# sakarias88/racer-tracer

Hardware: NVIDIA B200
Metric: samples/sec (higher is better)
Workload: dtype f32

## Files before the change

racer_tracer_b200/csrc/rc_api.cu:

```cuda
#include "../../include/racer_cuda.h"

#include <cmath>
#include <cstdio>
#include <cstdlib>
#include <cstring>
#include <chrono>
#include <map>
#include <string>
#include <thread>
#include <vector>

#include "rt_kernels.cuh"
#include "rt_wavefront.cuh"
#include <algorithm>

#include "rc_multi.cuh"
#include "rc_lbvh.cuh"
#include "rc_spec.cuh"

namespace {

thread_local std::string g_last_error;

int fail(int status, const std::string& msg) {
// ... 49 lines not shown
    cudaStream_t stream = nullptr;
    bool own_stream = true;
    cudaEvent_t ev0 = nullptr, ev1 = nullptr;
    cudaEvent_t ev_traced = nullptr;
    DevBuf<int> cancel_word;
    cudaStream_t cancel_stream = nullptr;
    DevBuf<DevPrim> prims;
    DevBuf<DevPrim> prims_lin;
    DevBuf<DevNode> nodes;
    DevBuf<DevTexture> textures;
    DevBuf<DevInstance> instances;
    DevBuf<float4> perlin;
    DevBuf<uint8_t> perm;
    DevBuf<DevPrimD> prims_d;
    DevBuf<int> prim_kind;
    DevBuf<uint32_t> prim_id;
    DevBuf<DevNodeD> nodes_d;
    DevBuf<int> prim_inst;
    DevBuf<DevInstanceD> instances_d;
    std::vector<cudaArray_t> arrays;
    std::vector<std::pair<int, int>> array_dims;
    std::vector<cudaTextureObject_t> tex;
    DevBuf<float> accum;
    DevBuf<float> slice_buf;
    DevBuf<double> out64;
    DevBuf<double> pp_in, pp_mapped;
    DevBuf<uint8_t> pp_rgba;
    DevBuf<unsigned long long> counter;
    DevBuf<uint8_t> ad_active;
    DevBuf<int> ad_spp;
    DevBuf<float> ad_m2;
    DevBuf<double> ad_s2, ad_err;
    WavefrontState wf;
    std::map<std::string, SpecKernel> spec_cache;
    int sm_count = 0, clock_khz = 0;
};

}

struct rc_frame {
    float* base = nullptr;
    size_t image_floats = 0;
    int* words = nullptr;
    int width = 0, height = 0, rank = 0, world = 1;
    int frame_no = 0;
    bool owner = false;
    int* timed_out = nullptr;
// ... 161 lines not shown
    if (!instanced && s->n_prims <= RT_MAX_CONST_PRIMS && rects_fit) mode = RT_MODE_CONST_LINEAR;
    else if (s->n_nodes > 0 && bvh_bytes + perlin_bytes <= RC_SMEM_STAGE_LIMIT) mode = RT_MODE_SMEM_BVH;
    else if (s->n_nodes > 0) mode = RT_MODE_GLOBAL_BVH;
    else mode = RT_MODE_SMEM_LINEAR;
    if (force && !instanced) {
        std::string f(force);
        if (f == "const" && s->n_prims <= RT_MAX_CONST_PRIMS && rects_fit) mode = RT_MODE_CONST_LINEAR;
        else if (f == "smem" && s->n_nodes > 0) mode = RT_MODE_SMEM_BVH;
        else if (f == "global" && s->n_nodes > 0) mode = RT_MODE_GLOBAL_BVH;
        else if (f == "smemlin") mode = RT_MODE_SMEM_LINEAR;
    }
    smem_bytes = perlin_bytes;
    if (mode == RT_MODE_SMEM_BVH) smem_bytes += bvh_bytes;
    if (mode == RT_MODE_SMEM_LINEAR || mode == RT_MODE_CONST_LINEAR) smem_bytes += (size_t)s->n_prims * sizeof(DevPrim);
    return mode;
}

template <typename K>
int set_smem(K kernel, size_t bytes) {
    if (bytes > 48 * 1024) CUDA_TRY(cudaFuncSetAttribute(kernel, cudaFuncAttributeMaxDynamicSharedMemorySize, (int)bytes));
    return RC_OK;
}

template <int MODE, bool TEX>
int launch_mega_mode(const KParams& kp, float* accum, int sampler, int rounds, int blocks, size_t smem, cudaStream_t st) {
#define RC_LAUNCH(S, R)                                                                         \
    do {                                                                                        \
        int rc__ = set_smem(megakernel_render<MODE, S, R, TEX>, smem);                          \
        if (rc__ != RC_OK) return rc__;                                                         \
        megakernel_render<MODE, S, R, TEX><<<blocks, RT_BLOCK, smem, st>>>(kp, accum);          \
    } while (0)
    if (rounds == 7) { if (sampler == RC_SAMPLER_REJECTION) RC_LAUNCH(1, 7); else RC_LAUNCH(0, 7); }
    else { if (sampler == RC_SAMPLER_REJECTION) RC_LAUNCH(1, 10); else RC_LAUNCH(0, 10); }
#undef RC_LAUNCH
    CUDA_TRY(cudaGetLastError());
    return RC_OK;
}

template <int MODE, bool TEX>
int launch_moments_mode(const KParams& kp, float* accum, int blocks, size_t smem, cudaStream_t st, const uint8_t* active, float* round_m2) {
    int rc = set_smem(megakernel_moments<MODE, TEX>, smem);
    if (rc != RC_OK) return rc;
    megakernel_moments<MODE, TEX><<<blocks, RT_BLOCK, smem, st>>>(kp, accum, active, round_m2);
    CUDA_TRY(cudaGetLastError());
    return RC_OK;
}

int launch_mega(int mode, bool tex, const KParams& kp, float* accum, int sampler, int rounds, int blocks, size_t smem, cudaStream_t st,
                const uint8_t* active = nullptr, float* round_m2 = nullptr) {
#define RC_MODE(M) (!active ? (tex ? launch_mega_mode<M, true>(kp, accum, sampler, rounds, blocks, smem, st)          \
                                   : launch_mega_mode<M, false>(kp, accum, sampler, rounds, blocks, smem, st))        \
                             : (tex ? launch_moments_mode<M, true>(kp, accum, blocks, smem, st, active, round_m2)     \
                                    : launch_moments_mode<M, false>(kp, accum, blocks, smem, st, active, round_m2)))
    switch (mode) {
    case RT_MODE_CONST_LINEAR: return RC_MODE(RT_MODE_CONST_LINEAR);
    case RT_MODE_SMEM_BVH: return RC_MODE(RT_MODE_SMEM_BVH);
    case RT_MODE_GLOBAL_BVH: return RC_MODE(RT_MODE_GLOBAL_BVH);
    default: return RC_MODE(RT_MODE_SMEM_LINEAR);
    }
#undef RC_MODE
}

int check_params(const rc_params* p) {
    if (!p) return fail(RC_ERR_INVALID, "params is NULL");
    if (p->width < 2 || p->height < 2) return fail(RC_ERR_INVALID, "width and height must be >= 2 (u = x/(W-1), cpu.rs:35-40)");
    if (p->samples < 1) return fail(RC_ERR_INVALID, "samples must be >= 1");
    if (p->max_depth < 0) return fail(RC_ERR_INVALID, "max_depth must be >= 0");
    if (p->world < 0 || p->rank < 0 || (p->world > 0 && p->rank >= p->world)) return fail(RC_ERR_INVALID, "bad rank/world");
    if (p->rng_rounds != 0 && p->rng_rounds != 7 && p->rng_rounds != 10) return fail(RC_ERR_INVALID, "rng_rounds must be 0, 7 or 10");
    if ((long long)p->width * p->height > (1 << 24)) return fail(RC_ERR_INVALID, "more than 2^24 pixels (RNG counter layout)");
    if (p->samples > (1 << 24)) return fail(RC_ERR_INVALID, "more than 2^24 samples per pixel (RNG counter layout)");
    if (p->max_depth > 63) return fail(RC_ERR_INVALID, "max_depth > 63 (RNG counter layout)");
    if (p->variant != RC_VARIANT_MEGAKERNEL && p->variant != RC_VARIANT_WAVEFRONT) return fail(RC_ERR_INVALID, "unknown variant");
    if (p->sampler != RC_SAMPLER_DIRECT && p->sampler != RC_SAMPLER_REJECTION) return fail(RC_ERR_INVALID, "unknown sampler");
    if (p->split != RC_SPLIT_TILES && p->split != RC_SPLIT_SAMPLES) return fail(RC_ERR_INVALID, "unknown split");
    if (p->specialize < 0 || p->specialize > 2) return fail(RC_ERR_INVALID, "specialize must be 0, 1 or 2");
    if (!(p->tile_w == 0 && p->tile_h == 0) && !(p->tile_w == RT_TILE_W && p->tile_h == RT_TILE_H))
        return fail(RC_ERR_INVALID, "tile_w x tile_h must be 0 x 0 or 16 x 8 (the kernels' tile is fixed)");
    return RC_OK;
}

void set_vstep(KParams& kp, int screen_height) {
    const double s = 1.0 / ((double)(screen_height - 1) * 65536.0);
    kp.vstep = make_float4((float)(kp.cam.vertical.x * s), (float)(kp.cam.vertical.y * s), (float)(kp.cam.vertical.z * s), 0.0f);
}

void partition(KParams& kp, const rc_params* p, int part, int parts) {
    kp.width = p->width; kp.height = p->height;
    kp.max_depth = p->max_depth;
    kp.fixed_jitter = p->fixed_jitter;
    kp.key = (uint32_t)p->seed ^ (uint32_t)(p->seed >> 32);
    for (int r = 0; r < 10; ++r) kp.ks[r] = kp.key + (uint32_t)r * PHILOX2_W;
    kp.inv_wm1 = 1.0f / (float)(p->width - 1); kp.inv_hm1 = 1.0f / (float)(p->height - 1);
    kp.wm1 = (float)(p->width - 1);
    set_vstep(kp, p->height);
    kp.px_scale_x = kp.px_scale_y = 1;
    kp.tile_w = RT_TILE_W; kp.tile_h = RT_TILE_H;
    kp.slices = 1; kp.slice_buf = nullptr;
    kp.overwrite = 0;
    kp.final_scale = 0.0f;
    kp.tiles_x = (p->width + RT_TILE_W - 1) / RT_TILE_W;
    int tiles_y = (p->height + RT_TILE_H - 1) / RT_TILE_H;
    int total = kp.tiles_x * tiles_y;
    if (p->split == RC_SPLIT_SAMPLES) {
        kp.tile_first = 0; kp.tile_stride = 1; kp.n_tiles = total;
        long long lo = (long long)p->samples * part / parts, hi = (long long)p->samples * (part + 1) / parts;
        kp.s_begin = (int)lo; kp.s_end = (int)hi;
    } else {
        kp.tile_first = part; kp.tile_stride = parts;
        kp.n_tiles = part < total ? (total - part + parts - 1) / parts : 0;
        kp.s_begin = 0; kp.s_end = p->samples;
    }
}

bool cancelled(const volatile int32_t* cancel) { return cancel && *cancel != 0; }

bool direct_tiles(const rc_ctx* ctx, const rc_params* p) {
    return ctx->devs.size() > 1 && p->split == RC_SPLIT_TILES && ctx->multi.peer_write_ok && p->variant == RC_VARIANT_MEGAKERNEL;
}

struct AdaptiveRound {
    const uint8_t* active;
    float* round_m2;
    int s_begin, s_end;
};

struct ShareCall {
    float* accum0;
    const volatile int32_t* cancel;
    bool store = false;
    float final_scale = 0.0f;
    bool spread_stores = false;
    int preview_sw = 0, preview_sh = 0, preview_w = 0, preview_h = 0;
    const AdaptiveRound* round = nullptr;
};

int trace_share(rc_ctx* ctx, const rc_params* p, const ShareCall& call, bool& was_cancelled) {
    was_cancelled = false;
    const int n_dev = (int)ctx->devs.size();
    const int world = p->world > 0 ? p->world : 1;
    const int parts = world * n_dev;
    const int rounds = p->rng_rounds ? p->rng_rounds : 10;
    const bool direct = direct_tiles(ctx, p);
    uint64_t launches = 0;
    bool used_spec = false;
    for (int k = 0; k < n_dev; ++k) {
        DeviceState& d = ctx->devs[k];
        CUDA_TRY(cudaSetDevice(d.device));
        if (k == 0) {
            if (!call.round) CUDA_TRY(cudaEventRecord(d.ev0, d.stream));
            if (n_dev > 1) CUDA_TRY(cudaEventRecord(d.ev_traced, d.stream));
        } else {
            CUDA_TRY(cudaStreamWaitEvent(d.stream, ctx->devs[0].ev_traced, 0));
        }
        if (!call.round) CUDA_TRY(cudaMemsetAsync(d.counter.p, 0, sizeof(unsigned long long), d.stream));
    }
    const bool relay = call.cancel != nullptr && p->variant == RC_VARIANT_MEGAKERNEL;
    if (relay)
// ... 38 lines not shown
            continue;
        }
        SpecKernel* spec = nullptr;
        const bool spec_mode_ok = ctx->smem_bytes <= 48 * 1024 &&
                                  (ctx->mode == RT_MODE_CONST_LINEAR ||
                                   ((ctx->mode == RT_MODE_SMEM_BVH || ctx->mode == RT_MODE_GLOBAL_BVH) && std::getenv("RC_NO_BVH_SPEC") == nullptr));
        if (p->specialize && spec_mode_ok && p->sampler == RC_SAMPLER_DIRECT && !p->fixed_jitter) {
            std::string err;
            if (!spec_load_api((const void*)&rc_abi_version)) err = spec_api().err;
            else {
                if (ctx->spec_rounds != rounds) { ctx->spec_source.clear(); ctx->spec_source_moments.clear(); }
                std::string& source = call.round ? ctx->spec_source_moments : ctx->spec_source;
                if (source.empty()) {
                    source = spec_generate(ctx->kp, ctx->has_textures, ctx->mats_mask, ctx->mode, ctx->prims_mask, ctx->instanced, rounds,
                                           call.round != nullptr);
                    ctx->spec_rounds = rounds;
                }
                spec = spec_build(d.spec_cache, source, err, ++ctx->spec_clock);
            }
            if (!spec && p->specialize == 1) return fail(RC_ERR_STATE, "scene specialisation failed: " + err);
        } else if (p->specialize == 1) {
            return fail(RC_ERR_INVALID, "specialize = 1 needs the megakernel, the direct sampler and no fixed jitter");
        }
        const int s0 = kp.s_begin, s1 = kp.s_end;
        kp.slices = 1;
        kp.slice_buf = nullptr;
        kp.slice_halving = 0;
        if (!call.round) {
            const long long want = 8LL * d.sm_count * 10;
            long long sl = (want + kp.n_tiles - 1) / kp.n_tiles;
            if (sl > (s1 - s0) / 16) sl = (s1 - s0) / 16;
            if (sl < 2 && s1 - s0 >= 512 && !call.spread_stores) sl = 2;
            if (const char* e = std::getenv("RC_SLICES")) sl = std::atoll(e);
            kp.slice_halving = sl >= 5 ? 1 : 0;
            if (const char* e = std::getenv("RC_SLICE_HALVING")) kp.slice_halving = std::atoi(e);
            while (kp.slice_halving && sl > 1 && ((s1 - s0) >> (sl - 1)) < 8) --sl;
            if (sl > 1) {
                CUDA_TRY(d.slice_buf.resize((size_t)sl * kp.n_tiles * RT_BLOCK * 3));
                kp.slices = (int)sl;
                kp.slice_buf = d.slice_buf.p;
            }
        }
        {
            int rc = RC_ERR_CUDA;
            if (spec) {
                rc = spec_launch(spec, kp, accum, kp.n_tiles * kp.slices, ctx->smem_bytes, d.stream, active, round_m2) == 0 ? RC_OK : RC_ERR_CUDA;
                if (rc == RC_OK) used_spec = true;
                else if (p->specialize == 1) return fail(rc, "launch of the scene-specialised kernel failed");
            }
            if (rc != RC_OK)
                rc = launch_mega(ctx->mode, ctx->has_textures, kp, accum, p->sampler, rounds, kp.n_tiles * kp.slices, ctx->smem_bytes, d.stream,
                                 active, round_m2);
            if (rc != RC_OK) return rc;
            ++launches;
            if (kp.slices > 1) {
                reduce_slices_kernel<<<(kp.n_tiles * RT_BLOCK + 255) / 256, 256, 0, d.stream>>>(kp, accum);
                CUDA_TRY(cudaGetLastError());
                ++launches;
            }
        }
        if (relay) CUDA_TRY(cudaEventRecord(d.ev_traced, d.stream));
    }
    ctx->stats.kernel_launches = launches;
    ctx->stats.specialized = used_spec ? 1 : 0;
    if (relay) {
        for (;;) {
            bool done = true;
            for (int k = 0; k < n_dev && done; ++k) {
                const cudaError_t e = cudaEventQuery(ctx->devs[k].ev_traced);
                if (e == cudaErrorNotReady) done = false;
                else if (e != cudaSuccess) return fail(RC_ERR_CUDA, std::string("cudaEventQuery: ") + cudaGetErrorString(e));
            }
            if (!was_cancelled && cancelled(call.cancel)) {
                was_cancelled = true;
                for (int k = 0; k < n_dev; ++k) {
                    DeviceState& d = ctx->devs[k];
                    CUDA_TRY(cudaSetDevice(d.device));
                    CUDA_TRY(cudaMemcpyAsync(d.cancel_word.p, ctx->cancel_relay, sizeof(int), cudaMemcpyHostToDevice, d.cancel_stream));
                }
// ... 459 lines not shown
    for (int k = 0; k < n; ++k) {
        DeviceState& d = ctx->devs[k];
        d.device = devices ? devices[k] : k;
        if (d.device < 0 || d.device >= count) {
            delete ctx;
            return fail(RC_ERR_NO_DEVICE, "device ordinal out of range");
        }
        cudaError_t err = cudaSetDevice(d.device);
        if (err == cudaSuccess) err = cudaStreamCreateWithFlags(&d.stream, cudaStreamNonBlocking);
        if (err == cudaSuccess) err = cudaEventCreate(&d.ev0);
        if (err == cudaSuccess) err = cudaEventCreate(&d.ev1);
        if (err == cudaSuccess) err = cudaEventCreateWithFlags(&d.ev_traced, cudaEventDisableTiming);
        if (err == cudaSuccess) err = d.counter.resize(1);
        cudaDeviceProp prop;
        if (err == cudaSuccess) err = cudaGetDeviceProperties(&prop, d.device);
        if (err != cudaSuccess) {
            delete ctx;
            return fail(RC_ERR_CUDA, std::string("device setup failed: ") + cudaGetErrorString(err));
        }
        d.sm_count = prop.multiProcessorCount;
        d.clock_khz = prop.clockRate;
        {
            cudaFuncAttributes fa;
            cudaFuncGetAttributes(&fa, reduce_slices_kernel);
            cudaFuncGetAttributes(&fa, finalize_kernel);
            cudaFuncGetAttributes(&fa, finalize_to_f64_kernel);
            cudaFuncGetAttributes(&fa, widen_kernel);
            cudaFuncGetAttributes(&fa, frame_wait_kernel);
            cudaFuncGetAttributes(&fa, frame_publish_kernel);
            cudaFuncGetAttributes(&fa, sum_slots_kernel);
            cudaGetLastError();
        }
    }
    ctx->stats.n_devices = n;
    ctx->stats.sm_count = ctx->devs[0].sm_count;
    ctx->stats.sm_clock_khz = ctx->devs[0].clock_khz;
    int rc = multi_init(ctx->multi, ctx->devs.size(), [&](size_t k) { return ctx->devs[k].device; });
    if (rc != RC_OK) {
        delete ctx;
        return fail(rc, "peer access setup failed");
    }
    cudaSetDevice(ctx->devs[0].device);
    if (cudaHostAlloc((void**)&ctx->cancel_relay, sizeof(int), cudaHostAllocPortable) != cudaSuccess) {
        cudaGetLastError();
        rc_destroy(ctx);
        return fail(RC_ERR_CUDA, "cudaHostAlloc of the cancel relay failed");
    }
// ... 4 lines not shown
            cudaGetLastError();
            rc_destroy(ctx);
            return fail(RC_ERR_CUDA, "cudaStreamCreate of the cancel stream failed");
        }
    }
    cudaSetDevice(ctx->devs[0].device);
    *out = ctx;
    return RC_OK;
}

int rc_destroy(rc_ctx* ctx) {
    if (!ctx) return RC_OK;
    cudaSetDevice(ctx->devs.empty() ? 0 : ctx->devs[0].device);
    while (!ctx->frames.empty()) rc_frame_close(ctx, ctx->frames.back());
    for (void* q : ctx->shared_opened) cudaIpcCloseMemHandle(q);
    for (void* q : ctx->shared_owned) cudaFree(q);
    if (ctx->cancel_relay) cudaFreeHost(ctx->cancel_relay);
    multi_destroy(ctx->multi);
    for (auto& d : ctx->devs) {
        cudaSetDevice(d.device);
        cudaDeviceSynchronize();
        free_scene(d);
        free_tables(d);
        d.accum.release(); d.slice_buf.release(); d.out64.release(); d.counter.release(); d.cancel_word.release();
        d.ad_active.release(); d.ad_spp.release(); d.ad_m2.release(); d.ad_s2.release(); d.ad_err.release();
        if (d.cancel_stream) cudaStreamDestroy(d.cancel_stream);
        d.pp_in.release(); d.pp_mapped.release(); d.pp_rgba.release();
        if (d.ev_traced) cudaEventDestroy(d.ev_traced);
        wavefront_release(d.wf);
        spec_release(d.spec_cache);
        if (d.ev0) cudaEventDestroy(d.ev0);
        if (d.ev1) cudaEventDestroy(d.ev1);
        if (d.own_stream && d.stream) cudaStreamDestroy(d.stream);
    }
    delete ctx;
    return RC_OK;
}

int rc_set_stream(rc_ctx* ctx, void* cuda_stream) {
    if (!ctx) return fail(RC_ERR_INVALID, "ctx is NULL");
    DeviceState& d = ctx->devs[0];
    CUDA_TRY(cudaSetDevice(d.device));
    if (d.own_stream && d.stream) CUDA_TRY(cudaStreamDestroy(d.stream));
    d.stream = reinterpret_cast<cudaStream_t>(cuda_stream);
    d.own_stream = false;
    return RC_OK;
}
// ... 268 lines not shown
    if (p->variant != RC_VARIANT_MEGAKERNEL) return fail(RC_ERR_INVALID, "rc_render_frame needs the megakernel");
    const bool by_samples = p->split == RC_SPLIT_SAMPLES;
    if (p->width != f->width || p->height != f->height) return fail(RC_ERR_INVALID, "params and frame sizes differ");
    const int world = p->world > 0 ? p->world : 1;
    if (world != f->world || p->rank != f->rank) return fail(RC_ERR_INVALID, "params and frame rank / world differ");
    if (f->rank != 0 && (d_rgb || out_rgb)) return fail(RC_ERR_INVALID, "only rank 0 receives the image");
    if (ctx->devs.size() != 1) return fail(RC_ERR_INVALID, "rc_render_frame is the one-process-per-GPU form: the context must hold one device");
    if (!ctx->has_scene || !ctx->has_camera) return fail(RC_ERR_STATE, "upload a scene and set a camera first");
    if (cancelled(cancel)) return fail(RC_ERR_CANCELLED, "cancel flag set before the render started");
    if (*f->timed_out) return fail(RC_ERR_STATE, "an earlier frame never completed (a rank stopped publishing progress)");
    DeviceState& d = ctx->devs[0];
    CUDA_TRY(cudaSetDevice(d.device));
    const int frame_no = ++f->frame_no;
    float* image = f->base + (size_t)(frame_no & 1) * f->world * f->image_floats;
    float* target = by_samples ? image + (size_t)f->rank * f->image_floats : image;
    if (world > 1) {
        if (f->rank == 0) frame_publish_kernel<<<1, 1, 0, d.stream>>>(f->words, frame_no + 1);
        else frame_wait_kernel<<<1, 32, 0, d.stream>>>(f->words, 0, 1, frame_no, f->timed_out);
        CUDA_TRY(cudaGetLastError());
    }
    bool was_cancelled = false;
    ShareCall call{target, cancel, true};
    call.final_scale = by_samples ? 0.0f : 1.0f / (float)p->samples;
    call.spread_stores = by_samples && world > 1;
    rc = trace_share(ctx, p, call, was_cancelled);
    if (rc != RC_OK) return rc;
    if (by_samples && (long long)p->samples * (f->rank + 1) / world <= (long long)p->samples * f->rank / world) {
        CUDA_TRY(cudaMemsetAsync(target, 0, f->image_floats * sizeof(float), d.stream));
    }
    uint64_t extra = 0;
    if (world > 1) {
        if (f->rank != 0) { frame_publish_kernel<<<1, 1, 0, d.stream>>>(f->words + 32 * f->rank, frame_no); extra = 2; }
        else { frame_wait_kernel<<<1, 32, 0, d.stream>>>(f->words, 1, world - 1, frame_no, f->timed_out); extra = 2; }
        CUDA_TRY(cudaGetLastError());
    }
    if (by_samples && f->rank == 0) {
        const size_t n = (size_t)p->width * p->height * 3;
        sum_slots_kernel<<<(unsigned)((n + 255) / 256), 256, 0, d.stream>>>(image, f->image_floats, world, n, 1.0f / (float)p->samples);
        CUDA_TRY(cudaGetLastError());
        extra += 1;
    }
    rc = finish_stats(ctx, p);
    if (rc != RC_OK) return rc;
    ctx->stats.kernel_launches += extra;
    if (d_rgb) *d_rgb = image;
    if (out_rgb && !was_cancelled) {
        const size_t n = (size_t)p->width * p->height * 3;
// ... 432 lines not shown
```

racer_tracer_b200/csrc/rc_spec.cuh:

```cuda
#pragma once
#include <cuda_runtime.h>
#include <dlfcn.h>

#include <cmath>
#include <cstdio>
#include <cstdlib>
#include <cstring>
#include <fstream>
#include <map>
#include <sstream>
#include <string>
#include <vector>

#include "rt_kernels.cuh"

struct SpecKernel {
    void* module = nullptr;
    void* function = nullptr;
    std::string source;
    std::string error;
    uint64_t last_use = 0;
};

#define RC_SPEC_CACHE_MAX 8

struct SpecApi {
    bool tried = false, ok = false;
    std::string err;
    void* nvrtc = nullptr;
    void* cuda = nullptr;
    int (*CreateProgram)(void**, const char*, const char*, int, const char* const*, const char* const*) = nullptr;
    int (*CompileProgram)(void*, int, const char* const*) = nullptr;
    int (*GetCUBINSize)(void*, size_t*) = nullptr;
    int (*GetCUBIN)(void*, char*) = nullptr;
    int (*GetProgramLogSize)(void*, size_t*) = nullptr;
    int (*GetProgramLog)(void*, char*) = nullptr;
    int (*DestroyProgram)(void**) = nullptr;
    int (*cuModuleLoadData)(void**, const void*) = nullptr;
    int (*cuModuleGetFunction)(void**, void*, const char*) = nullptr;
    int (*cuModuleUnload)(void*) = nullptr;
    int (*cuLaunchKernel)(void*, unsigned, unsigned, unsigned, unsigned, unsigned, unsigned, unsigned, void*, void**, void**) = nullptr;
    std::string header_dir;
};

inline SpecApi& spec_api() {
    static SpecApi api;
    return api;
}

inline bool spec_load_api(const void* anchor_symbol) {
    SpecApi& a = spec_api();
    if (a.tried) return a.ok;
    a.tried = true;
    const char* nvrtc_names[] = {"libnvrtc.so.12", "libnvrtc.so", "/usr/local/cuda/lib64/libnvrtc.so.12"};
    for (const char* n : nvrtc_names) { a.nvrtc = dlopen(n, RTLD_NOW); if (a.nvrtc) break; }
    if (!a.nvrtc) { a.err = "libnvrtc.so.12 not found"; return false; }
    a.cuda = dlopen("libcuda.so.1", RTLD_NOW);
    if (!a.cuda) { a.err = "libcuda.so.1 not found"; return false; }
#define RC_SYM(lib, field, name)                                                        \
    *(void**)(&a.field) = dlsym(a.lib, name);                                           \
    if (!a.field) { a.err = std::string("missing symbol ") + name; return false; }
    RC_SYM(nvrtc, CreateProgram, "nvrtcCreateProgram");
    RC_SYM(nvrtc, CompileProgram, "nvrtcCompileProgram");
    RC_SYM(nvrtc, GetCUBINSize, "nvrtcGetCUBINSize");
    RC_SYM(nvrtc, GetCUBIN, "nvrtcGetCUBIN");
    RC_SYM(nvrtc, GetProgramLogSize, "nvrtcGetProgramLogSize");
    RC_SYM(nvrtc, GetProgramLog, "nvrtcGetProgramLog");
    RC_SYM(nvrtc, DestroyProgram, "nvrtcDestroyProgram");
    RC_SYM(cuda, cuModuleLoadData, "cuModuleLoadData");
    RC_SYM(cuda, cuModuleGetFunction, "cuModuleGetFunction");
    RC_SYM(cuda, cuModuleUnload, "cuModuleUnload");
    RC_SYM(cuda, cuLaunchKernel, "cuLaunchKernel");
#undef RC_SYM
    Dl_info info;
    if (!dladdr(anchor_symbol, &info) || !info.dli_fname) { a.err = "cannot locate the library on disk"; return false; }
    std::string path(info.dli_fname);
    size_t slash = path.find_last_of('/');
    a.header_dir = (slash == std::string::npos ? std::string(".") : path.substr(0, slash)) + "/csrc/";
    a.ok = true;
    return true;
}

inline int __float_as_int_host(float f) { int i; std::memcpy(&i, &f, sizeof(i)); return i; }

inline std::string spec_float(float v) {
    char buf[64];
    std::snprintf(buf, sizeof(buf), "%.9g", (double)v);
    std::string s(buf);
    if (s.find_first_of(".eEn") == std::string::npos) s += ".0";
    return s + "f";
}

inline std::string spec_entry(const char* mode, int rounds, bool tex, bool moments) {
    std::ostringstream o;
    o << "extern \"C\" __global__ void __launch_bounds__(RT_BLOCK, RT_MIN_BLOCKS)\n"
// ... 393 lines not shown
        return remember_failure();
    }
    size_t n = 0;
    a.GetCUBINSize(prog, &n);
    std::vector<char> cubin(n);
    a.GetCUBIN(prog, cubin.data());
    a.DestroyProgram(&prog);
    SpecKernel k;
    k.source = source;
    k.last_use = now;
    if (a.cuModuleLoadData(&k.module, cubin.data()) != 0) { err = "cuModuleLoadData failed"; return remember_failure(); }
    if (a.cuModuleGetFunction(&k.function, k.module, "spec_megakernel") != 0) { err = "spec_megakernel not found in module"; return remember_failure(); }
    auto res = cache.emplace(source, k);
    return &res.first->second;
}

inline void spec_release(std::map<std::string, SpecKernel>& cache) {
    SpecApi& a = spec_api();
    for (auto& kv : cache)
        if (kv.second.module && a.cuModuleUnload) a.cuModuleUnload(kv.second.module);
    cache.clear();
}

inline int spec_launch(SpecKernel* k, const KParams& kp, float* accum, int blocks, size_t smem, cudaStream_t st,
                       const uint8_t* active = nullptr, float* round_m2 = nullptr) {
    SpecApi& a = spec_api();
    KParams p = kp;
    void* args[4] = {&p, &accum, &active, &round_m2};
    return a.cuLaunchKernel(k->function, (unsigned)blocks, 1, 1, RT_BLOCK, 1, 1, (unsigned)smem, (void*)st, args, nullptr);
}
```

racer_tracer_b200/csrc/rt_kernels.cuh:

```cuda
#pragma once
#include "rt_scene.cuh"

#define RT_TILE_W 16
#define RT_TILE_H 8
#define RT_BLOCK 128

#define RT_MODE_CONST_LINEAR 0
#define RT_MODE_SMEM_BVH 1
#define RT_MODE_GLOBAL_BVH 2
#define RT_MODE_SMEM_LINEAR 3

struct SmemLayout {
    const DevNode* nodes;
    const DevPrim* prims;
    const float4* perlin;
    const uint8_t* perm;
};

template <int MODE>
RT_D SmemLayout stage_scene(const KParams& P, unsigned char* smem) {
    SmemLayout L;
    L.nodes = P.nodes; L.prims = P.prims; L.perlin = P.perlin; L.perm = P.perlin_perm;
    float4* dst = reinterpret_cast<float4*>(smem);
    if (MODE == RT_MODE_SMEM_BVH) {
// ... 231 lines not shown

#ifndef RT_STEAL
#define RT_STEAL 1
#endif
#ifndef RT_STEAL_MIN
#define RT_STEAL_MIN 4
#endif


#ifndef RT_KCONST_MASK
#define RT_KCONST_MASK 7
#endif
#ifndef RT_PHILOX_LATE
#define RT_PHILOX_LATE 0
#endif

RT_D float radiance_y(const vec3f& a, const vec3f& b) { return (a.x * b.x + a.y * b.y + a.z * b.z) * (1.0f / 3.0f); }

template <int MODE, int SAMPLER, int ROUNDS, bool TEX, bool MOMENTS = false>
RT_D void megakernel_body(const KParams& P, float* __restrict__ accum, unsigned char* smem,
                          const uint8_t* __restrict__ active_px = nullptr, float* __restrict__ round_m2 = nullptr) {
    constexpr int PARKED = MOMENTS ? 4 : 3;
    __shared__ float steal_parked[RT_STEAL ? PARKED * RT_BLOCK : 1];
    if (P.cancel_flag != nullptr &&
        __syncthreads_or(threadIdx.x == 0 && *reinterpret_cast<const volatile int*>(P.cancel_flag) != 0)) return;
    bool active = true;
    if constexpr (MOMENTS) {
        const int tile = P.tile_first + (int)blockIdx.x * P.tile_stride;
        const int w = threadIdx.x >> 5, l = threadIdx.x & 31;
        const int x = (tile % P.tiles_x) * RT_TILE_W + (w & 1) * 8 + (l & 7);
        const int y = (tile / P.tiles_x) * RT_TILE_H + (w >> 1) * 4 + (l >> 3);
        active = x < P.width && y < P.height && active_px[y * P.width + x] != 0;
        if (!__syncthreads_or(active ? 1 : 0)) return;
    }
    __shared__ float reg_consts[7];
    if (threadIdx.x == 0) {
        reg_consts[0] = 2.0f; reg_consts[1] = 6.283185307179586f / 16777216.0f; reg_consts[2] = 1.0f;
#ifdef RT_SPECIALIZED
        spec_reg_consts(reg_consts + 3);
#endif
    }
    SmemLayout L = stage_scene<MODE>(P, smem);
    TexCtx X; X.perlin = L.perlin; X.perm = L.perm;
    {
        const volatile float* rc = reg_consts;
        if (RT_KCONST_MASK & 1) X.k_two = rc[0];
        if (RT_KCONST_MASK & 2) X.k_phi = rc[1];
        if (RT_KCONST_MASK & 4) X.k_one = rc[2];
#ifdef RT_SPECIALIZED
#pragma unroll
        for (int j = 0; j < RT_SPEC_REG_CONSTS; ++j) X.k_spec[j] = rc[3 + j];
#endif
    }

    const int slice = P.slices > 1 ? (int)blockIdx.x / P.n_tiles : 0;
    const int tile_k = P.slices > 1 ? (int)blockIdx.x - slice * P.n_tiles : (int)blockIdx.x;
    const int tile = P.tile_first + tile_k * P.tile_stride;
    const int tx = tile % P.tiles_x, ty = tile / P.tiles_x;
    const int warp = threadIdx.x >> 5, lane = threadIdx.x & 31;
    const int px = tx * RT_TILE_W + (warp & 1) * 8 + (lane & 7);
    const int py = ty * RT_TILE_H + (warp >> 1) * 4 + (lane >> 3);
    const bool valid = px < P.width && py < P.height;
    int s_first = P.s_begin, s_last = P.s_end;
    if (P.slices > 1 && P.slice_halving) {
        const int n = P.s_end - P.s_begin;
        s_first = P.s_begin + (n - (n >> slice));
        s_last = slice + 1 == P.slices ? P.s_end : P.s_begin + (n - (n >> (slice + 1)));
    } else if (P.slices > 1) {
        const long long n = P.s_end - P.s_begin, S = P.slices, total = S * (S + 1) / 2;
        const long long c0 = (long long)slice * S - (long long)slice * (slice - 1) / 2;
        const long long c1 = c0 + (S - slice);
        s_first = P.s_begin + (int)(n * c0 / total);
        s_last = P.s_begin + (int)(n * c1 / total);
    }

    PixelCtx pc = pixel_setup<ROUNDS>(P, valid ? px : 0, valid ? py : 0);
    RngCtx R; R.ks = P.ks; R.pixel = pc.pixel; R.sample = 0;
    const uint32_t own_pixel = pc.pixel;
    PhiloxPre ppre = philox2x32_pre(pc.pixel, P.ks);
    uint32_t vj_bits = __byte_perm(0u, 0u, 0);
    {
        const uint2 w = philox2x32_from<ROUNDS>(ppre, rt_ctr1(rt_vjit_sample((uint32_t)s_first), 0u, RT_TAG_PATH), P.ks);
        vj_bits = __byte_perm(w.y, w.x, 0x0040);
    }
    int owner = lane;
    float* const parked = steal_parked + 32 * PARKED * warp;
    if (RT_STEAL) {
        parked[lane] = 0.0f; parked[lane + 32] = 0.0f; parked[lane + 64] = 0.0f;
        if constexpr (MOMENTS) parked[lane + 96] = 0.0f;
        __syncwarp();
    }

    vec3f sum = mk3(0.0f, 0.0f, 0.0f);
    float m2 = 0.0f;
    vec3f o = mk3(0.0f, 0.0f, 0.0f), d = o, T = o;
    const vec3f T_ONE = mk3(1.0f, 1.0f, 1.0f);
    float time = 0.0f;
    int s = valid && active ? s_first : s_last;
    float depth_left = 0.0f;
    int last_prim = -1;
    uint32_t seg = 0;
    uint32_t ctr1 = 0;
    unsigned sh_prims = (unsigned)__cvta_generic_to_shared(L.prims);
    asm volatile("" : "+r"(sh_prims));
    unsigned nseg = 0;
    if (P.max_depth <= 0) {
        const float n = (float)(s_last - s);
        sum = mk3(n, n, n);
        if constexpr (MOMENTS) m2 = n;
        s = s_last;
    }

    if (P.tile_cull && (MODE == RT_MODE_CONST_LINEAR || MODE == RT_MODE_SMEM_LINEAR) && P.max_depth > 0) {
        if (!tile_may_hit(P, L.prims, tx, ty)) {
            if (valid) {
                nseg += (unsigned)(s_last - s);
#pragma unroll 1
                for (; s < s_last; ++s) {
                    if (RT_SPEC_BG_BLACK) { s = s_last; break; }
                    vec3f bg;
                    if (__float_as_int(P.bg_a.w) == 0) {
                        const uint2 rnd = philox2x32_ks<ROUNDS>(pc.pixel, rt_ctr1(rt_vjit_sample((uint32_t)s), 0u, RT_TAG_PATH), P.ks);
                        const float vjit = RT_FIXED_JITTER(P) ? 32768.0f : u16lo_int(rnd);
                        camera_ray<SAMPLER, ROUNDS>(P, pc, (uint32_t)s, vjit, o, d, time);
                        bg = background_color(P, d);
                    } else bg = mk3(P.bg_a.x, P.bg_a.y, P.bg_a.z);
                    sum = mk3(fmaf(T_ONE.x, bg.x, sum.x), fmaf(T_ONE.y, bg.y, sum.y), fmaf(T_ONE.z, bg.z, sum.z));
                    if constexpr (MOMENTS) { const float y = radiance_y(T_ONE, bg); m2 = fmaf(y, y, m2); }
                }
            }
            s = s_last;
        }
    }

#ifdef RT_SPEC_SNAP_TABLE
    __syncthreads();
    if ((int)threadIdx.x < P.n_prims) {
        float* row = const_cast<float*>(reinterpret_cast<const float*>(L.prims + threadIdx.x));
        float4 a = make_float4(0.f, 0.f, 0.f, 0.f);
        float bx = 0.f, cw = 0.f;
        spec_snap_row((int)threadIdx.x, a, bx, cw);
        row[0] = a.x; row[1] = a.y; row[2] = a.z; row[3] = a.w; row[4] = bx; row[11] = cw;
    }
    __syncthreads();
#endif

    auto iteration = [&]() {
        const bool fresh = depth_left == 0.0f;
        if (fresh) {
            R.sample = (uint32_t)s;
            ctr1 = R.sample;
            seg = 0; last_prim = -1;
            T = mk3(1.0f, 1.0f, 1.0f);
            depth_left = (float)P.max_depth;
        }
        asm("{\n\t.reg .pred pf;\n\tsetp.ne.s32 pf, %1, 0;\n\t@pf add.s32 %0, %0, 1;\n\t}" : "+r"(s) : "r"((int)fresh));
        if (fresh) {
            const float vjit = RT_FIXED_JITTER(P) ? 32768.0f : (float)(unsigned short)vj_bits;
            camera_ray<SAMPLER, ROUNDS>(P, pc, R.sample, vjit, o, d, time);
        }
#if !RT_PHILOX_LATE
        const uint2 rnd = philox2x32_from<ROUNDS>(ppre, ctr1, P.ks);
        if (fresh) vj_bits = __byte_perm(rnd.y, rnd.x, 0x0040);
#endif
        RayT<float> r = make_ray(o, d, time);
        float t;
        int prim;
        if (MODE == RT_MODE_CONST_LINEAR) { ConstScene S(P, sh_prims); prim = closest_hit<MODE>(P, S, r, last_prim, t, X); }
// ... 85 lines not shown
    }
#undef RT_LANE_BUSY
    if (RT_STEAL) {
        unsigned pending = __ballot_sync(0xffffffffu, owner != lane);
        while (pending) {
            const int l = __ffs(pending) - 1;
            pending &= pending - 1;
            if (lane == l) {
                parked[owner] += sum.x; parked[owner + 32] += sum.y; parked[owner + 64] += sum.z;
                if constexpr (MOMENTS) parked[owner + 96] += m2;
            }
            __syncwarp();
        }
        if (owner != lane) { sum = mk3(0.0f, 0.0f, 0.0f); m2 = 0.0f; }
        sum = mk3(sum.x + parked[lane], sum.y + parked[lane + 32], sum.z + parked[lane + 64]);
        if constexpr (MOMENTS) m2 += parked[lane + 96];
    }
    if constexpr (MOMENTS) {
        if (valid && active) {
            float* a = accum + 3 * (size_t)own_pixel;
            a[0] += sum.x; a[1] += sum.y; a[2] += sum.z;
            round_m2[own_pixel] = m2;
        }
    } else if (P.slices > 1) {
        float* a = P.slice_buf + 3 * ((size_t)slice * ((size_t)P.n_tiles * RT_BLOCK) + (size_t)tile_k * RT_BLOCK + threadIdx.x);
        a[0] = sum.x; a[1] = sum.y; a[2] = sum.z;
    } else if (valid) {
        float* a = accum + 3 * (size_t)own_pixel;
        if (P.final_scale != 0.0f) sum = mk3(sqrtf(P.final_scale * sum.x), sqrtf(P.final_scale * sum.y), sqrtf(P.final_scale * sum.z));
        if (P.overwrite) { a[0] = sum.x; a[1] = sum.y; a[2] = sum.z; }
        else { a[0] += sum.x; a[1] += sum.y; a[2] += sum.z; }
    }
    for (int off = 16; off > 0; off >>= 1) nseg += __shfl_xor_sync(0xffffffffu, nseg, off);
    if (lane == 0 && P.segment_counter) atomicAdd(P.segment_counter, (unsigned long long)nseg);
}

#ifndef RT_SPECIALIZED
__global__ void reduce_slices_kernel(const __grid_constant__ KParams P, float* __restrict__ accum) {
    const int rank = blockIdx.x * blockDim.x + threadIdx.x;
    if (rank >= P.n_tiles * RT_BLOCK) return;
    const int tile_k = rank / RT_BLOCK, within = rank % RT_BLOCK;
    const int tile = P.tile_first + tile_k * P.tile_stride;
    const int tx = tile % P.tiles_x, ty = tile / P.tiles_x;
    const int warp = within >> 5, lane = within & 31;
    const int px = tx * RT_TILE_W + (warp & 1) * 8 + (lane & 7);
    const int py = ty * RT_TILE_H + (warp >> 1) * 4 + (lane >> 3);
    if (px >= P.width || py >= P.height) return;
    float sx = 0.f, sy = 0.f, sz = 0.f;
    for (int j = 0; j < P.slices; ++j) {
        const float* a = P.slice_buf + 3 * ((size_t)j * ((size_t)P.n_tiles * RT_BLOCK) + rank);
        sx += a[0]; sy += a[1]; sz += a[2];
    }
    float* dst = accum + 3 * ((size_t)py * P.width + px);
    if (P.final_scale != 0.0f) { sx = sqrtf(P.final_scale * sx); sy = sqrtf(P.final_scale * sy); sz = sqrtf(P.final_scale * sz); }
    if (P.overwrite) { dst[0] = sx; dst[1] = sy; dst[2] = sz; }
    else { dst[0] += sx; dst[1] += sy; dst[2] += sz; }
}

template <int MODE, int SAMPLER, int ROUNDS, bool TEX>
__global__ void __launch_bounds__(RT_BLOCK, MODE == RT_MODE_GLOBAL_BVH ? RT_MIN_BLOCKS_GLOBAL_BVH : RT_MIN_BLOCKS)
megakernel_render(const __grid_constant__ KParams P, float* __restrict__ accum) {
    extern __shared__ __align__(16) unsigned char smem[];
    megakernel_body<MODE, SAMPLER, ROUNDS, TEX>(P, accum, smem);
}

template <int MODE, bool TEX>
__global__ void __launch_bounds__(RT_BLOCK, MODE == RT_MODE_GLOBAL_BVH ? RT_MIN_BLOCKS_GLOBAL_BVH : RT_MIN_BLOCKS)
megakernel_moments(const __grid_constant__ KParams P, float* __restrict__ accum, const uint8_t* __restrict__ active,
                   float* __restrict__ round_m2) {
    extern __shared__ __align__(16) unsigned char smem[];
    megakernel_body<MODE, 0, 10, TEX, true>(P, accum, smem, active, round_m2);
}

// ... 353 lines not shown
```

racer_tracer_b200/csrc/rt_scene.cuh:

```cuda
#pragma once
#include "rt_math.cuh"

#define RT_PRIM_SPHERE 0
#define RT_PRIM_XY 1
#define RT_PRIM_XZ 2
#define RT_PRIM_YZ 3
#define RT_PRIM_MOVING 4
#define RT_IS_SPHERE(type) (((type) & 3) == 0)
#define RT_MAT_LAMBERTIAN 0
#define RT_MAT_METAL 1
#define RT_MAT_DIELECTRIC 2
#define RT_MAT_LIGHT 3
#define RT_TEX_SOLID 0
#define RT_TEX_CHECKER 1
#define RT_TEX_IMAGE 2
#define RT_TEX_NOISE 3

#ifndef RT_SPEC_PRIMS
#define RT_SPEC_PRIMS 0xF
#endif
#ifndef RT_HAS_INSTANCES
#define RT_HAS_INSTANCES 1
#endif
#define RT_HAS_SPHERES (RT_SPEC_PRIMS & 1)
// ... 43 lines not shown

template <typename T>
struct DevCamera {
    Vec3T<T> origin, upper_left_corner, right, up, horizontal, vertical;
    T lens_radius, time_a, time_b;
};

struct KParams {
    DevCamera<float> cam;
    float4 bg_a, bg_b;
    int width, height;
    float inv_wm1, inv_hm1;
    float wm1;
    float4 vstep;
    int px_scale_x, px_scale_y;
    int s_begin, s_end;
    int max_depth;
    int fixed_jitter;
    uint32_t key;
    uint32_t ks[10];
    int tile_first, tile_stride, n_tiles;
    int overwrite;
    float final_scale;
    int slices;
    int slice_halving;
    float* slice_buf;
    int tiles_x, tile_w, tile_h;
    int n_prims, n_nodes;
    int lin_end[4];
    int n_perlin;
    int checker_depth;
    int lens_enabled;
    int tile_cull;
    int has_motion;
    int ref_aabb;
    const DevPrim* prims;
    const DevPrim* prims_lin;
    const DevNode* nodes;
    const DevTexture* textures;
    const DevInstance* instances;
    const float4* perlin;
    const uint8_t* perlin_perm;
    cudaTextureObject_t images[RT_MAX_IMAGES];
    int image_w[RT_MAX_IMAGES], image_h[RT_MAX_IMAGES];
    unsigned long long* segment_counter;
    const int* cancel_flag;
    DevPrim cprims[RT_MAX_CONST_PRIMS];
    float4 crect_bounds[3][RT_MAX_CONST_RECTS];
    float crect_k[3][RT_MAX_CONST_RECTS];
// ... 743 lines not shown
```

Measured before the change: 65.55 billion.

## Replace static sample slicing with persistent blocks pulling a dynamic work queue

Replaces the fixed per-tile sample slicing with a host-built work list. Tail tiles are split into sample-range pieces, and a persistent grid sized by occupancy takes items through an atomic counter. Each partial piece writes to its own slot, and a reduce-slots kernel sums the slots of cut tiles only. The goal is better load balancing at the tail and less launch and reduction overhead. The cost is an atomic and a block barrier per work item, plus host work-list construction that is cached by a key.

```diff
diff --git a/racer_tracer_b200/csrc/rc_api.cu b/racer_tracer_b200/csrc/rc_api.cu
--- a/racer_tracer_b200/csrc/rc_api.cu
+++ b/racer_tracer_b200/csrc/rc_api.cu
@@ -95,7 +95,10 @@
     std::vector<std::pair<int, int>> array_dims;
     std::vector<cudaTextureObject_t> tex;
     DevBuf<float> accum;
-    DevBuf<float> slice_buf;
+    DevBuf<int4> work;
+    std::vector<int4> work_items, work_cut;
+    int work_slots = 0;
+    long long work_key[5] = {-1, -1, -1, -1, -1};
     DevBuf<double> out64;
     DevBuf<double> pp_in, pp_mapped;
     DevBuf<uint8_t> pp_rgba;
@@ -303,13 +306,19 @@
     return RC_OK;
 }
 
+int persistent_grid(const KParams& kp, int blocks, int per_sm, int sm_count) {
+    return kp.n_items > 0 ? std::min(blocks, std::max(per_sm, 1) * sm_count) : blocks;
+}
+
 template <int MODE, bool TEX>
-int launch_mega_mode(const KParams& kp, float* accum, int sampler, int rounds, int blocks, size_t smem, cudaStream_t st) {
+int launch_mega_mode(const KParams& kp, float* accum, int sampler, int rounds, int blocks, int sm_count, size_t smem, cudaStream_t st) {
 #define RC_LAUNCH(S, R)                                                                         \
     do {                                                                                        \
         int rc__ = set_smem(megakernel_render<MODE, S, R, TEX>, smem);                          \
         if (rc__ != RC_OK) return rc__;                                                         \
-        megakernel_render<MODE, S, R, TEX><<<blocks, RT_BLOCK, smem, st>>>(kp, accum);          \
+        int per_sm__ = 0;                                                                       \
+        CUDA_TRY(cudaOccupancyMaxActiveBlocksPerMultiprocessor(&per_sm__, megakernel_render<MODE, S, R, TEX>, RT_BLOCK, smem)); \
+        megakernel_render<MODE, S, R, TEX><<<persistent_grid(kp, blocks, per_sm__, sm_count), RT_BLOCK, smem, st>>>(kp, accum); \
     } while (0)
     if (rounds == 7) { if (sampler == RC_SAMPLER_REJECTION) RC_LAUNCH(1, 7); else RC_LAUNCH(0, 7); }
     else { if (sampler == RC_SAMPLER_REJECTION) RC_LAUNCH(1, 10); else RC_LAUNCH(0, 10); }
@@ -319,20 +328,23 @@
 }
 
 template <int MODE, bool TEX>
-int launch_moments_mode(const KParams& kp, float* accum, int blocks, size_t smem, cudaStream_t st, const uint8_t* active, float* round_m2) {
+int launch_moments_mode(const KParams& kp, float* accum, int blocks, int sm_count, size_t smem, cudaStream_t st, const uint8_t* active,
+                        float* round_m2) {
     int rc = set_smem(megakernel_moments<MODE, TEX>, smem);
     if (rc != RC_OK) return rc;
-    megakernel_moments<MODE, TEX><<<blocks, RT_BLOCK, smem, st>>>(kp, accum, active, round_m2);
+    int per_sm = 0;
+    CUDA_TRY(cudaOccupancyMaxActiveBlocksPerMultiprocessor(&per_sm, megakernel_moments<MODE, TEX>, RT_BLOCK, smem));
+    megakernel_moments<MODE, TEX><<<persistent_grid(kp, blocks, per_sm, sm_count), RT_BLOCK, smem, st>>>(kp, accum, active, round_m2);
     CUDA_TRY(cudaGetLastError());
     return RC_OK;
 }
 
-int launch_mega(int mode, bool tex, const KParams& kp, float* accum, int sampler, int rounds, int blocks, size_t smem, cudaStream_t st,
-                const uint8_t* active = nullptr, float* round_m2 = nullptr) {
-#define RC_MODE(M) (!active ? (tex ? launch_mega_mode<M, true>(kp, accum, sampler, rounds, blocks, smem, st)          \
-                                   : launch_mega_mode<M, false>(kp, accum, sampler, rounds, blocks, smem, st))        \
-                             : (tex ? launch_moments_mode<M, true>(kp, accum, blocks, smem, st, active, round_m2)     \
-                                    : launch_moments_mode<M, false>(kp, accum, blocks, smem, st, active, round_m2)))
+int launch_mega(int mode, bool tex, const KParams& kp, float* accum, int sampler, int rounds, int blocks, int sm_count, size_t smem,
+                cudaStream_t st, const uint8_t* active = nullptr, float* round_m2 = nullptr) {
+#define RC_MODE(M) (!active ? (tex ? launch_mega_mode<M, true>(kp, accum, sampler, rounds, blocks, sm_count, smem, st)          \
+                                   : launch_mega_mode<M, false>(kp, accum, sampler, rounds, blocks, sm_count, smem, st))        \
+                             : (tex ? launch_moments_mode<M, true>(kp, accum, blocks, sm_count, smem, st, active, round_m2)     \
+                                    : launch_moments_mode<M, false>(kp, accum, blocks, sm_count, smem, st, active, round_m2)))
     switch (mode) {
     case RT_MODE_CONST_LINEAR: return RC_MODE(RT_MODE_CONST_LINEAR);
     case RT_MODE_SMEM_BVH: return RC_MODE(RT_MODE_SMEM_BVH);
@@ -377,7 +389,7 @@
     set_vstep(kp, p->height);
     kp.px_scale_x = kp.px_scale_y = 1;
     kp.tile_w = RT_TILE_W; kp.tile_h = RT_TILE_H;
-    kp.slices = 1; kp.slice_buf = nullptr;
+    kp.n_items = 0; kp.unused0 = 0; kp.work = nullptr;
     kp.overwrite = 0;
     kp.final_scale = 0.0f;
     kp.tiles_x = (p->width + RT_TILE_W - 1) / RT_TILE_W;
@@ -411,10 +423,30 @@
     const volatile int32_t* cancel;
     bool store = false;
     float final_scale = 0.0f;
-    bool spread_stores = false;
     int preview_sw = 0, preview_sh = 0, preview_w = 0, preview_h = 0;
     const AdaptiveRound* round = nullptr;
 };
+
+#define RC_MIN_PIECE 16
+
+void build_work_list(int n_tiles, int s0, int s1, int sm_count, long long forced, std::vector<int4>& items,
+                     std::vector<int4>& cut, int& n_slots) {
+    items.clear(); cut.clear(); n_slots = 0;
+    const long long n = s1 - s0, load = (long long)sm_count * RT_MIN_BLOCKS;
+    const long long tail = forced > 0 ? n_tiles : std::min<long long>(n_tiles, 2 * load);
+    for (int k = 0; k < n_tiles - tail; ++k) items.push_back(make_int4(k, 0, 0, -1));
+    for (long long k = n_tiles - tail; k < n_tiles; ++k) {
+        long long pieces = std::min(forced, n);
+        if (forced <= 0) {
+            const long long piece = std::max<long long>(RC_MIN_PIECE, (n_tiles - k) * n / (2 * load));
+            pieces = std::max<long long>(1, n / piece);
+        }
+        if (pieces <= 1) { items.push_back(make_int4((int)k, 0, 0, -1)); continue; }
+        cut.push_back(make_int4((int)k, n_slots, (int)pieces, 0));
+        for (long long j = 0; j < pieces; ++j)
+            items.push_back(make_int4((int)k, s0 + (int)(n * j / pieces), s0 + (int)(n * (j + 1) / pieces), n_slots++));
+    }
+}
 
 int trace_share(rc_ctx* ctx, const rc_params* p, const ShareCall& call, bool& was_cancelled) {
     was_cancelled = false;
@@ -499,39 +531,43 @@
         } else if (p->specialize == 1) {
             return fail(RC_ERR_INVALID, "specialize = 1 needs the megakernel, the direct sampler and no fixed jitter");
         }
-        const int s0 = kp.s_begin, s1 = kp.s_end;
-        kp.slices = 1;
-        kp.slice_buf = nullptr;
-        kp.slice_halving = 0;
-        if (!call.round) {
-            const long long want = 8LL * d.sm_count * 10;
-            long long sl = (want + kp.n_tiles - 1) / kp.n_tiles;
-            if (sl > (s1 - s0) / 16) sl = (s1 - s0) / 16;
-            if (sl < 2 && s1 - s0 >= 512 && !call.spread_stores) sl = 2;
-            if (const char* e = std::getenv("RC_SLICES")) sl = std::atoll(e);
-            kp.slice_halving = sl >= 5 ? 1 : 0;
-            if (const char* e = std::getenv("RC_SLICE_HALVING")) kp.slice_halving = std::atoi(e);
-            while (kp.slice_halving && sl > 1 && ((s1 - s0) >> (sl - 1)) < 8) --sl;
-            if (sl > 1) {
-                CUDA_TRY(d.slice_buf.resize((size_t)sl * kp.n_tiles * RT_BLOCK * 3));
-                kp.slices = (int)sl;
-                kp.slice_buf = d.slice_buf.p;
+        {
+            long long forced = call.round ? 1 : 0;
+            if (const char* e = std::getenv("RC_SLICES"); e && !call.round) forced = std::atoll(e);
+            const long long key[5] = {kp.n_tiles, forced == 1 ? 0 : kp.s_begin, forced == 1 ? 0 : kp.s_end, d.sm_count, forced};
+            if (!std::equal(key, key + 5, d.work_key)) {
+                build_work_list(kp.n_tiles, kp.s_begin, kp.s_end, d.sm_count, forced, d.work_items, d.work_cut, d.work_slots);
+                const size_t n_items = d.work_items.size(), slot_int4s = (size_t)d.work_slots * RT_BLOCK * 3 / 4;
+                CUDA_TRY(d.work.resize(1 + n_items + slot_int4s + d.work_cut.size()));
+                std::vector<int4> head(1 + n_items, make_int4(0, 0, 0, 0));
+                std::copy(d.work_items.begin(), d.work_items.end(), head.begin() + 1);
+                CUDA_TRY(cudaMemcpyAsync(d.work.p, head.data(), head.size() * sizeof(int4), cudaMemcpyHostToDevice, d.stream));
+                if (!d.work_cut.empty())
+                    CUDA_TRY(cudaMemcpyAsync(d.work.p + 1 + n_items + slot_int4s, d.work_cut.data(), d.work_cut.size() * sizeof(int4),
+                                             cudaMemcpyHostToDevice, d.stream));
+                std::copy(key, key + 5, d.work_key);
             }
-        }
+            kp.n_items = (int)d.work_items.size();
+            kp.work = d.work.p;
+        }
+        const int blocks = kp.n_items;
         {
             int rc = RC_ERR_CUDA;
             if (spec) {
-                rc = spec_launch(spec, kp, accum, kp.n_tiles * kp.slices, ctx->smem_bytes, d.stream, active, round_m2) == 0 ? RC_OK : RC_ERR_CUDA;
+                rc = spec_launch(spec, kp, accum, persistent_grid(kp, blocks, spec_blocks_per_sm(spec, ctx->smem_bytes), d.sm_count),
+                                 ctx->smem_bytes, d.stream, active, round_m2) == 0 ? RC_OK : RC_ERR_CUDA;
                 if (rc == RC_OK) used_spec = true;
                 else if (p->specialize == 1) return fail(rc, "launch of the scene-specialised kernel failed");
             }
             if (rc != RC_OK)
-                rc = launch_mega(ctx->mode, ctx->has_textures, kp, accum, p->sampler, rounds, kp.n_tiles * kp.slices, ctx->smem_bytes, d.stream,
+                rc = launch_mega(ctx->mode, ctx->has_textures, kp, accum, p->sampler, rounds, blocks, d.sm_count, ctx->smem_bytes, d.stream,
                                  active, round_m2);
             if (rc != RC_OK) return rc;
             ++launches;
-            if (kp.slices > 1) {
-                reduce_slices_kernel<<<(kp.n_tiles * RT_BLOCK + 255) / 256, 256, 0, d.stream>>>(kp, accum);
+            if (!d.work_cut.empty()) {
+                const int n_cut = (int)d.work_cut.size();
+                const int4* cut = d.work.p + 1 + d.work_items.size() + (size_t)d.work_slots * RT_BLOCK * 3 / 4;
+                reduce_slots_kernel<<<(n_cut * RT_BLOCK + 255) / 256, 256, 0, d.stream>>>(kp, accum, cut, n_cut);
                 CUDA_TRY(cudaGetLastError());
                 ++launches;
             }
@@ -1037,7 +1073,7 @@
         d.clock_khz = prop.clockRate;
         {
             cudaFuncAttributes fa;
-            cudaFuncGetAttributes(&fa, reduce_slices_kernel);
+            cudaFuncGetAttributes(&fa, reduce_slots_kernel);
             cudaFuncGetAttributes(&fa, finalize_kernel);
             cudaFuncGetAttributes(&fa, finalize_to_f64_kernel);
             cudaFuncGetAttributes(&fa, widen_kernel);
@@ -1088,7 +1124,7 @@
         cudaDeviceSynchronize();
         free_scene(d);
         free_tables(d);
-        d.accum.release(); d.slice_buf.release(); d.out64.release(); d.counter.release(); d.cancel_word.release();
+        d.accum.release(); d.work.release(); d.out64.release(); d.counter.release(); d.cancel_word.release();
         d.ad_active.release(); d.ad_spp.release(); d.ad_m2.release(); d.ad_s2.release(); d.ad_err.release();
         if (d.cancel_stream) cudaStreamDestroy(d.cancel_stream);
         d.pp_in.release(); d.pp_mapped.release(); d.pp_rgba.release();
@@ -1403,7 +1439,6 @@
     bool was_cancelled = false;
     ShareCall call{target, cancel, true};
     call.final_scale = by_samples ? 0.0f : 1.0f / (float)p->samples;
-    call.spread_stores = by_samples && world > 1;
     rc = trace_share(ctx, p, call, was_cancelled);
     if (rc != RC_OK) return rc;
     if (by_samples && (long long)p->samples * (f->rank + 1) / world <= (long long)p->samples * f->rank / world) {
diff --git a/racer_tracer_b200/csrc/rc_spec.cuh b/racer_tracer_b200/csrc/rc_spec.cuh
--- a/racer_tracer_b200/csrc/rc_spec.cuh
+++ b/racer_tracer_b200/csrc/rc_spec.cuh
@@ -40,6 +40,7 @@
     int (*cuModuleGetFunction)(void**, void*, const char*) = nullptr;
     int (*cuModuleUnload)(void*) = nullptr;
     int (*cuLaunchKernel)(void*, unsigned, unsigned, unsigned, unsigned, unsigned, unsigned, unsigned, void*, void**, void**) = nullptr;
+    int (*cuOccupancyMaxActiveBlocksPerMultiprocessor)(int*, void*, int, size_t) = nullptr;
     std::string header_dir;
 };
 
@@ -71,6 +72,7 @@
     RC_SYM(cuda, cuModuleGetFunction, "cuModuleGetFunction");
     RC_SYM(cuda, cuModuleUnload, "cuModuleUnload");
     RC_SYM(cuda, cuLaunchKernel, "cuLaunchKernel");
+    RC_SYM(cuda, cuOccupancyMaxActiveBlocksPerMultiprocessor, "cuOccupancyMaxActiveBlocksPerMultiprocessor");
 #undef RC_SYM
     Dl_info info;
     if (!dladdr(anchor_symbol, &info) || !info.dli_fname) { a.err = "cannot locate the library on disk"; return false; }
@@ -510,6 +512,11 @@
     cache.clear();
 }
 
+inline int spec_blocks_per_sm(SpecKernel* k, size_t smem) {
+    int n = 0;
+    return spec_api().cuOccupancyMaxActiveBlocksPerMultiprocessor(&n, k->function, RT_BLOCK, smem) == 0 ? n : 0;
+}
+
 inline int spec_launch(SpecKernel* k, const KParams& kp, float* accum, int blocks, size_t smem, cudaStream_t st,
                        const uint8_t* active = nullptr, float* round_m2 = nullptr) {
     SpecApi& a = spec_api();
diff --git a/racer_tracer_b200/csrc/rt_kernels.cuh b/racer_tracer_b200/csrc/rt_kernels.cuh
--- a/racer_tracer_b200/csrc/rt_kernels.cuh
+++ b/racer_tracer_b200/csrc/rt_kernels.cuh
@@ -277,17 +277,6 @@
                           const uint8_t* __restrict__ active_px = nullptr, float* __restrict__ round_m2 = nullptr) {
     constexpr int PARKED = MOMENTS ? 4 : 3;
     __shared__ float steal_parked[RT_STEAL ? PARKED * RT_BLOCK : 1];
-    if (P.cancel_flag != nullptr &&
-        __syncthreads_or(threadIdx.x == 0 && *reinterpret_cast<const volatile int*>(P.cancel_flag) != 0)) return;
-    bool active = true;
-    if constexpr (MOMENTS) {
-        const int tile = P.tile_first + (int)blockIdx.x * P.tile_stride;
-        const int w = threadIdx.x >> 5, l = threadIdx.x & 31;
-        const int x = (tile % P.tiles_x) * RT_TILE_W + (w & 1) * 8 + (l & 7);
-        const int y = (tile / P.tiles_x) * RT_TILE_H + (w >> 1) * 4 + (l >> 3);
-        active = x < P.width && y < P.height && active_px[y * P.width + x] != 0;
-        if (!__syncthreads_or(active ? 1 : 0)) return;
-    }
     __shared__ float reg_consts[7];
     if (threadIdx.x == 0) {
         reg_consts[0] = 2.0f; reg_consts[1] = 6.283185307179586f / 16777216.0f; reg_consts[2] = 1.0f;
@@ -308,25 +297,50 @@
 #endif
     }
 
-    const int slice = P.slices > 1 ? (int)blockIdx.x / P.n_tiles : 0;
-    const int tile_k = P.slices > 1 ? (int)blockIdx.x - slice * P.n_tiles : (int)blockIdx.x;
+#ifdef RT_SPEC_SNAP_TABLE
+    if ((int)threadIdx.x < P.n_prims) {
+        float* row = const_cast<float*>(reinterpret_cast<const float*>(L.prims + threadIdx.x));
+        float4 a = make_float4(0.f, 0.f, 0.f, 0.f);
+        float bx = 0.f, cw = 0.f;
+        spec_snap_row((int)threadIdx.x, a, bx, cw);
+        row[0] = a.x; row[1] = a.y; row[2] = a.z; row[3] = a.w; row[4] = bx; row[11] = cw;
+    }
+    __syncthreads();
+    const DevPrim* const cull_prims = P.prims_lin;
+#else
+    const DevPrim* const cull_prims = L.prims;
+#endif
+
+    __shared__ int item_sh[2];
+#pragma unroll 1
+    for (int k = 0;; ++k) {
+    int tile_k, s_first, s_last, slot;
+    {
+        if (threadIdx.x == 0) {
+            int* const counter = &P.work[0].x;
+            const volatile int* const cancel = P.cancel_flag;
+            int it;
+            do it = atomicAdd(counter, 1); while (it < P.n_items && cancel != nullptr && *cancel != 0);
+            if (it == P.n_items + (int)gridDim.x - 1) atomicExch(counter, 0);
+            item_sh[k & 1] = it;
+        }
+        __syncthreads();
+        const int it = item_sh[k & 1];
+        if (it >= P.n_items) break;
+        const int4 w = P.work[1 + it];
+        tile_k = w.x; slot = w.w;
+        s_first = slot < 0 ? P.s_begin : w.y; s_last = slot < 0 ? P.s_end : w.z;
+    }
     const int tile = P.tile_first + tile_k * P.tile_stride;
     const int tx = tile % P.tiles_x, ty = tile / P.tiles_x;
     const int warp = threadIdx.x >> 5, lane = threadIdx.x & 31;
     const int px = tx * RT_TILE_W + (warp & 1) * 8 + (lane & 7);
     const int py = ty * RT_TILE_H + (warp >> 1) * 4 + (lane >> 3);
     const bool valid = px < P.width && py < P.height;
-    int s_first = P.s_begin, s_last = P.s_end;
-    if (P.slices > 1 && P.slice_halving) {
-        const int n = P.s_end - P.s_begin;
-        s_first = P.s_begin + (n - (n >> slice));
-        s_last = slice + 1 == P.slices ? P.s_end : P.s_begin + (n - (n >> (slice + 1)));
-    } else if (P.slices > 1) {
-        const long long n = P.s_end - P.s_begin, S = P.slices, total = S * (S + 1) / 2;
-        const long long c0 = (long long)slice * S - (long long)slice * (slice - 1) / 2;
-        const long long c1 = c0 + (S - slice);
-        s_first = P.s_begin + (int)(n * c0 / total);
-        s_last = P.s_begin + (int)(n * c1 / total);
+    bool active = true;
+    if constexpr (MOMENTS) {
+        active = valid && active_px[py * P.width + px] != 0;
+        if (!__syncthreads_or(active ? 1 : 0)) continue;
     }
 
     PixelCtx pc = pixel_setup<ROUNDS>(P, valid ? px : 0, valid ? py : 0);
@@ -367,7 +381,7 @@
     }
 
     if (P.tile_cull && (MODE == RT_MODE_CONST_LINEAR || MODE == RT_MODE_SMEM_LINEAR) && P.max_depth > 0) {
-        if (!tile_may_hit(P, L.prims, tx, ty)) {
+        if (!tile_may_hit(P, cull_prims, tx, ty)) {
             if (valid) {
                 nseg += (unsigned)(s_last - s);
 #pragma unroll 1
@@ -387,18 +401,6 @@
             s = s_last;
         }
     }
-
-#ifdef RT_SPEC_SNAP_TABLE
-    __syncthreads();
-    if ((int)threadIdx.x < P.n_prims) {
-        float* row = const_cast<float*>(reinterpret_cast<const float*>(L.prims + threadIdx.x));
-        float4 a = make_float4(0.f, 0.f, 0.f, 0.f);
-        float bx = 0.f, cw = 0.f;
-        spec_snap_row((int)threadIdx.x, a, bx, cw);
-        row[0] = a.x; row[1] = a.y; row[2] = a.z; row[3] = a.w; row[4] = bx; row[11] = cw;
-    }
-    __syncthreads();
-#endif
 
     auto iteration = [&]() {
         const bool fresh = depth_left == 0.0f;
@@ -530,8 +532,8 @@
             a[0] += sum.x; a[1] += sum.y; a[2] += sum.z;
             round_m2[own_pixel] = m2;
         }
-    } else if (P.slices > 1) {
-        float* a = P.slice_buf + 3 * ((size_t)slice * ((size_t)P.n_tiles * RT_BLOCK) + (size_t)tile_k * RT_BLOCK + threadIdx.x);
+    } else if (slot >= 0) {
+        float* a = reinterpret_cast<float*>(P.work + 1 + P.n_items) + 3 * ((size_t)slot * RT_BLOCK + threadIdx.x);
         a[0] = sum.x; a[1] = sum.y; a[2] = sum.z;
     } else if (valid) {
         float* a = accum + 3 * (size_t)own_pixel;
@@ -541,22 +543,25 @@
     }
     for (int off = 16; off > 0; off >>= 1) nseg += __shfl_xor_sync(0xffffffffu, nseg, off);
     if (lane == 0 && P.segment_counter) atomicAdd(P.segment_counter, (unsigned long long)nseg);
+    }
 }
 
 #ifndef RT_SPECIALIZED
-__global__ void reduce_slices_kernel(const __grid_constant__ KParams P, float* __restrict__ accum) {
+__global__ void reduce_slots_kernel(const __grid_constant__ KParams P, float* __restrict__ accum, const int4* __restrict__ cut, int n_cut) {
     const int rank = blockIdx.x * blockDim.x + threadIdx.x;
-    if (rank >= P.n_tiles * RT_BLOCK) return;
-    const int tile_k = rank / RT_BLOCK, within = rank % RT_BLOCK;
-    const int tile = P.tile_first + tile_k * P.tile_stride;
+    if (rank >= n_cut * RT_BLOCK) return;
+    const int4 c = cut[rank / RT_BLOCK];
+    const int within = rank % RT_BLOCK;
+    const int tile = P.tile_first + c.x * P.tile_stride;
     const int tx = tile % P.tiles_x, ty = tile / P.tiles_x;
     const int warp = within >> 5, lane = within & 31;
     const int px = tx * RT_TILE_W + (warp & 1) * 8 + (lane & 7);
     const int py = ty * RT_TILE_H + (warp >> 1) * 4 + (lane >> 3);
     if (px >= P.width || py >= P.height) return;
     float sx = 0.f, sy = 0.f, sz = 0.f;
-    for (int j = 0; j < P.slices; ++j) {
-        const float* a = P.slice_buf + 3 * ((size_t)j * ((size_t)P.n_tiles * RT_BLOCK) + rank);
+    const float* slots = reinterpret_cast<const float*>(P.work + 1 + P.n_items);
+    for (int j = c.y; j < c.y + c.z; ++j) {
+        const float* a = slots + 3 * ((size_t)j * RT_BLOCK + within);
         sx += a[0]; sy += a[1]; sz += a[2];
     }
     float* dst = accum + 3 * ((size_t)py * P.width + px);
diff --git a/racer_tracer_b200/csrc/rt_scene.cuh b/racer_tracer_b200/csrc/rt_scene.cuh
--- a/racer_tracer_b200/csrc/rt_scene.cuh
+++ b/racer_tracer_b200/csrc/rt_scene.cuh
@@ -89,9 +89,9 @@
     int tile_first, tile_stride, n_tiles;
     int overwrite;
     float final_scale;
-    int slices;
-    int slice_halving;
-    float* slice_buf;
+    int n_items;
+    int unused0;
+    int4* work;
     int tiles_x, tile_w, tile_h;
     int n_prims, n_nodes;
     int lin_end[4];
```

After: 63.33 billion, median of 6. -3.4%, worse.
